# yfukasawa/LongQC

Measured on AMD Instinct MI355X. Metric: Mbases/sec all-vs-all overlap coverage (sampleqc hot path), higher is better.
Workload: dtype u64; 1 GPU; BASELINE configs[2]: 500000 synthetic PacBio Sequel CLR reads ~10 kb 30x, pb-sequel preset (-Y -l 0 -q 160 -k 12 -w 5 -I 4G -p 80), 5000 subsample queries; target_bases=5181693140, query_bases=51577117, parallelism=single GPU

## Files before the change

longqc_amd/csrc/engine.cpp:

```cpp
#include "engine.hpp"
#include "kernels_sketch.hpp"
#include "kernels_index.hpp"
#include "kernels_seed.hpp"
#include "kernels_sort.hpp"
#include "kernels_walk.hpp"
#include "kernels_psort.hpp"
#include "kernels_chain.hpp"
#include "fastx.hpp"
#include "fastx_mem.hpp"
#include "sat_replay.hpp"
#ifndef LQ_EMU
extern "C" void lq_segv_altstack();
#endif
#include <cstdio>
#include <cstring>
#include <cmath>
#include <cinttypes>
#include <algorithm>
#include <unordered_map>
#include <deque>
#include <future>
#include <functional>

static inline u32 nblk(u64 n, u32 bs)
// ... 50 lines not shown
}
void lqcov_handle::drain_stages()
{
	std::lock_guard<std::mutex> g(stage_mu);
	for (lqcov_handle::StagePending &sp : stage_pending) { hipEventSynchronize(sp.b); account_stage(sp.name, sp.a, sp.b, sp.bytes); }
	stage_pending.clear();
	for (auto &kv : late_bytes) { auto it = stages.find(kv.first); if (it != stages.end()) it->second.bytes += kv.second; }
	late_bytes.clear();
}
void lqcov_handle::add_stage_bytes(const char *name, u64 bytes)
{
	if (!profiling || !bytes) return;
	std::lock_guard<std::mutex> g(stage_mu);
	late_bytes[name] += bytes;
}

void Knobs::read_env()
{
	auto num = [](const char *name, long dflt) { const char *e = getenv(name); return e && *e ? atol(e) : dflt; };
	auto is = [](const char *name, const char *val) { const char *e = getenv(name); return e && !strcmp(e, val); };
	lanes = (int)std::min<long>(8, std::max<long>(1, num("LQCOV_LANES", 3)));
	anchor_budget = getenv("LQCOV_ANCHOR_BUDGET") ? strtoull(getenv("LQCOV_ANCHOR_BUDGET"), 0, 10) : 0;
	query_order_file = is("LQCOV_QUERY_ORDER", "file");
	query_order_striped = is("LQCOV_QUERY_ORDER", "striped");
	all_klib = is("LQCOV_SORT", "klib");
	ps_shift = (u32)std::min<long>(12, std::max<long>(0, num("LQCOV_PS_SHIFT", 0)));
	reg_walker = !is("LQCOV_WALK", "solo");
	ckpt = !is("LQCOV_CKPT", "0");
	ckpt3 = num("LQCOV_CKPT3", 1) > 0;
	sort_tile = (u32)std::max<long>(0, num("LQCOV_SORT_TILE", 0)); if (sort_tile && sort_tile < 64) sort_tile = 64;
	walk_shift = (u32)std::min<long>(16, std::max<long>(0, num("LQCOV_WALK_SHIFT", 0)));
	chain_wave_min = (int)std::max<long>(0, num("LQCOV_CHAIN_WAVE_MIN", 0));
	chain_cap = (int)num("LQCOV_CHAIN_CAP", 128);
	run_stage = (u32)std::max<long>(1, num("LQCOV_RUN_STAGE", LQ_RUN_STAGE));
	run_grid = (u32)std::max<long>(1, num("LQCOV_RUN_GRID", 2048));
	ps_key64 = num("LQCOV_PS_KEY64", 0) != 0;
	sketch_wgen = num("LQCOV_SKETCH_WGEN", 0) != 0;
	upload_amb = num("LQCOV_UPLOAD_AMB", 0) != 0;
	sketch_fast = num("LQCOV_SKETCH_FAST", 1) != 0;
#ifndef LQ_EMU
	lq_trace_launches = (int)num("LQCOV_TRACE_LAUNCHES", 0);
#endif
	no_level_skip = getenv("LQCOV_NO_LEVEL_SKIP") != nullptr;
	debug_sort = getenv("LQCOV_DEBUG_SORT") != nullptr;
	sketch_kpt = (u32)std::min<long>(64, std::max<long>(1, num("LQCOV_SKETCH_KPT", 4)));
	sketch_machine_only = is("LQCOV_SKETCH", "machine");
	upload_slices = (u32)std::min<long>(8, std::max<long>(1, num("LQCOV_UPLOAD_SLICES", 4)));
	upload_min_chunks = (u64)std::max<long>(1, num("LQCOV_UPLOAD_MIN_CHUNKS", 1L << 16));
	tile_grid = (u32)std::max<long>(64, num("LQCOV_TILE_GRID", 4096));
	ps_passes = (u32)std::min<long>(16, std::max<long>(0, num("LQCOV_PS_PASSES", 2))) & ~1u;
	ties_klib = is("LQCOV_TIES", "klib") || all_klib;
	filter = num("LQCOV_FILTER", 1) != 0;
	parse_threads = (int)std::min<long>(256, std::max<long>(0, num("LQCOV_PARSE_THREADS", 0)));
	parse_piece = (u64)std::max<long>(64, num("LQCOV_PARSE_PIECE", 32L << 20));
	parse_side = getenv("LQCOV_PARSE_SIDE") ? strtoull(getenv("LQCOV_PARSE_SIDE"), 0, 10) : 2ULL << 30;
	pipeline = num("LQCOV_PIPELINE", 1) != 0;
	plan_ahead = num("LQCOV_PLAN_AHEAD", 1) != 0;
	cnt_bits = (int)std::min<long>(16, std::max<long>(2, num("LQCOV_TEST_CNT_BITS", 16)));
	seed_bucket = (u32)std::min<long>(1L << 24, std::max<long>(16, num("LQCOV_SEED_BUCKET", 7600)));
	seed_chunk = getenv("LQCOV_SEED_CHUNK") ? std::max<u64>(1024, strtoull(getenv("LQCOV_SEED_CHUNK"), 0, 10)) : 1ULL << 30;
	if (seed_chunk > 0xfffffff0ULL) seed_chunk = 0xfffffff0ULL;
	seed_segl = (u32)std::min<long>(LQ_SD_SEGL, std::max<long>(1, num("LQCOV_SEED_SEGL", LQ_SD_SEGL)));
	seed_pair_bits = (u32)std::min<long>(LQ_SD_PAIR_BITS, std::max<long>(1, num("LQCOV_SEED_PAIR_BITS", LQ_SD_PAIR_BITS)));
	seed_hwords = (u32)std::min<long>(LQ_SD_HWORDS, std::max<long>(2, num("LQCOV_SEED_HWORDS", LQ_SD_HWORDS)));
	seed_surv_max = getenv("LQCOV_SEED_SURV_MAX") ? std::max<u64>(1, strtoull(getenv("LQCOV_SEED_SURV_MAX"), 0, 10)) : 2ULL << 30;
	seed_dcap = (u32)std::min<long>(LQ_SD_DCAP, std::max<long>(1, num("LQCOV_SEED_DCAP", LQ_SD_DCAP)));
// ... 709 lines not shown
		sort_recs.push_back(std::move(rec));
	}
	if (K.debug_sort) {
		std::vector<mm128> ha(nA);
		d2h(ha.data(), dA, nA, L.stream);
		u64 sum_after = 0;
		for (u64 i = 0; i < nA; ++i) sum_after += dbg_anchor_sum(ha[i]);
		if (sum_after != sum_before) fprintf(stderr, "[sort] batch of %u queries: NOT A PERMUTATION of the emitted anchors (sums %016llx / %016llx)\n", nqb, (unsigned long long)sum_before, (unsigned long long)sum_after);
		u64 unsorted = 0, ties = 0, unmarked = 0;
		for (u32 q = 0; q < nqb; ++q)
			for (u64 i = h_off[q] + 1; i < h_off[q + 1]; ++i) {
				if (ha[i].x < ha[i - 1].x) ++unsorted;
				if (ha[i].x == ha[i - 1].x) { ++ties; if (!(ha[i].y & LQ_TIE_MARK) || !(ha[i - 1].y & LQ_TIE_MARK)) { if (unmarked++ < 4) fprintf(stderr, "[sort] query %u of the batch: equal x %016llx, y %016llx / %016llx\n", q, (unsigned long long)ha[i].x, (unsigned long long)ha[i - 1].y, (unsigned long long)ha[i].y); } }
			}
		fprintf(stderr, "[sort] batch of %u queries: %llu anchors, %llu out of order, %llu equal-x neighbours, %llu of them with an unmarked anchor\n", nqb, (unsigned long long)nA, (unsigned long long)unsorted, (unsigned long long)ties, (unsigned long long)unmarked);
		if (sum_after != sum_before || unsorted || unmarked) throw std::logic_error("LQCOV_DEBUG_SORT: the sorted anchors are not a permutation of the emitted ones, not ascending, or hold an unmarked tie (see stderr)");
	}
}

void lqcov_handle::batch_buffers(MapLane &L, u64 nA)
{
	if (nA > 0xfffffff0ULL) throw std::domain_error("a single query produces more than 2^32 anchors against this part");
	const u64 nA4 = ((nA + 1) * 4 + 15) & ~(u64)15;
	L.A.ensure((nA + 1) * 16); L.B.ensure(std::max<u64>((nA + 1) * 16, nA4 * 4));
	L.scr.ensure(nA4 * 5 + 64);
}

void lqcov_handle::chain_stage(MapLane &L, Part &pt, const u64 *aqb, u64 a_base, u32 nqb, u32 q0, const u32 *qmap, u64 nA, int tie_mode, u32 n_want, u32 ivl_cap, bool dbg, const SatSink *sink)
{
	mm128 *dA = L.A.as<mm128>();
	const u64 nA4 = ((nA + 1) * 4 + 15) & ~(u64)15;
	u64 *d_cu = (u64*)((u8*)L.scr.p + 3 * nA4);
	i32 *d_cf = (i32*)L.B.p, *d_cp = (i32*)((u8*)L.B.p + nA4), *d_ct = (i32*)((u8*)L.B.p + 2 * nA4), *d_cv = (i32*)((u8*)L.B.p + 3 * nA4);
	u64 n_groups = 0;
	if (tie_mode == 2 && a_base == 0 && qmap) {
		L.gstart.ensure(((u64)n_want + 1) * 8);
		if (n_want) {
			StageTimer t(this, L.stream, "k_run_list", (u64)n_want * 16);
			LQ_LAUNCH(k_want_runs, nblk(n_want, 256), 256, L.stream, dA, aqb, nqb, qmap, L.want.as<unsigned long long>(), n_want, L.gstart.as<u64>()); check_launch();
		}
		n_groups = n_want;
	} else {
		const u32 n_tiles = (u32)((nA + LQ_RUN_TILE - 1) / LQ_RUN_TILE);
		const u32 n_min = run_n_min();
		L.run_tiles.ensure(16);
		L.gstart.ensure((nA / n_min + 1) * 8);
		dzero(L.run_tiles.p, 4, L.stream);
		{
			StageTimer t(this, L.stream, "k_run_list", nA * 16);
			LQ_LAUNCH(k_run_list, std::min<u32>(n_tiles, K.run_grid), LQ_RUN_THREADS, L.stream, dA, nA, aqb, a_base, nqb, n_tiles, n_min, std::max<u32>(LQ_RUN_THREADS, std::min<u32>(K.run_stage, LQ_RUN_STAGE)), L.run_tiles.as<u32>(), L.gstart.as<u64>()); check_launch();
		}
		u32 ng = 0;
		d2h(&ng, L.run_tiles.as<u32>(), 1, L.stream);
		n_groups = ng;
	}
	ChainBufs cb; cb.f = d_cf; cb.p = d_cp; cb.t = d_ct; cb.v = d_cv; cb.u = d_cu;
	CovState cs;
	cs.lambda = lambda.as<unsigned long long>(); cs.lambda2 = lambda2.as<unsigned long long>();
	cs.cnts = cnts.as<u32>(); cs.qflags = qflags.as<u32>(); cs.skip = skip.as<u32>(); cs.qmoff = cnt_off_dev();
	cs.mini_pos = mini_pos.as<u64>(); cs.mpq_off = mpq_off.as<u64>(); cs.qlen = q.d_len.as<u32>(); cs.tlen = pt.rs.d_len.as<u32>();
	cs.ivl = L.ivl.as<Ivl>(); cs.n_ivl = L.n_ivl.as<u32>(); cs.ivl_cap = ivl_cap;
	cs.dbg = dbg ? dbg_chains.as<ChainRec>() : nullptr; cs.n_dbg = n_dbg.as<unsigned long long>(); cs.dbg_cap = dbg_cap;
	cs.tie_mode = tie_mode; cs.qmap = qmap; cs.thr = have_thr ? q_thr.as<u32>() : nullptr;
	cs.cnt_max = cnt_max;
	cs.rec = sink ? sink->rec : nullptr; cs.n_rec = sink ? sink->n_rec : nullptr; cs.rec_cap = sink ? sink->rec_cap : 0;
	cs.rec_at = sink ? sink->at : nullptr; cs.n_at = sink ? sink->n_at : nullptr; cs.at_cap = sink ? sink->at_cap : 0;
	cs.sens = nullptr; cs.n_sens = L.n_sens.as<u32>(); cs.sens_cap = 0; cs.want = L.want.as<unsigned long long>(); cs.n_want = n_want;
	if (tie_mode == 1) {
		L.sens.ensure((n_groups + 1) * 8);
		cs.sens = L.sens.as<unsigned long long>(); cs.sens_cap = (u32)std::min<u64>(n_groups, 0xfffffff0ULL);
	}
	if (n_groups > 0xfffffff0ULL) throw std::domain_error("too many anchor runs in one batch");
	const int cap = K.chain_cap <= 64 ? 64 : K.chain_cap <= 128 ? 128 : 256;
	const int wave_min = tie_mode == 2 && K.chain_wave_min <= 0 ? std::min<int>(LQ_CHAIN_WAVE_MIN, std::max<int>(P.min_cnt, 8)) : std::min(cap + 1, K.chain_wave_min > 0 ? K.chain_wave_min : LQ_CHAIN_WAVE_MIN);
	if (n_groups) {
		StageTimer t(this, L.stream, "k_chain", nA * 16);
#define LQ_CHAIN_LAUNCH(CAP) LQ_LAUNCH((k_chain<CAP>), nblk(n_groups, 64), 64, L.stream, dA, L.gstart.as<u64>(), (const u32*)nullptr, (u32)n_groups, aqb, a_base, nqb, q0, avg_qspan.as<float>(), mp, cs, (i32)P.min_cnt, (i32)(wave_min - 1))
		if (cap == 64) { LQ_CHAIN_LAUNCH(64); } else if (cap == 128) { LQ_CHAIN_LAUNCH(128); } else { LQ_CHAIN_LAUNCH(256); }
#undef LQ_CHAIN_LAUNCH
		check_launch();
	}
	{
		u32 n_sel = 0;
		const u32 n_tiles = (u32)((n_groups + LQ_RUN_TILE - 1) / LQ_RUN_TILE);
		L.sel_tiles.ensure(((u64)n_tiles + 2) * 4);
		LQ_LAUNCH(k_sel_count, std::min<u32>(std::max<u32>(n_tiles, 1), 1u << 16), LQ_RUN_THREADS, L.stream, L.gstart.as<u64>(), n_groups, (i32)wave_min, (i32)0x7fffffff, n_tiles, L.sel_tiles.as<u32>()); check_launch();
		LQ_LAUNCH(k_tile_scan, 1, LQ_TSCAN_THREADS, L.stream, L.sel_tiles.as<u32>(), n_tiles); check_launch();
		d2h(&n_sel, L.sel_tiles.as<u32>() + n_tiles, 1, L.stream);
		if (n_sel) {
			L.gsel.ensure((u64)n_sel * 4); L.gkey.ensure((u64)n_sel * 4); L.gsel2.ensure((u64)n_sel * 4); L.gkey2.ensure((u64)n_sel * 4);
			LQ_LAUNCH(k_sel_write, std::min<u32>(n_tiles, 1u << 16), LQ_RUN_THREADS, L.stream, L.gstart.as<u64>(), n_groups, (i32)wave_min, (i32)0x7fffffff, n_tiles, L.sel_tiles.as<u32>(), L.gsel.as<u32>(), L.gkey.as<u32>()); check_launch();
			L.prim.sort_pairs_u32_u32(L.gkey.as<u32>(), L.gkey2.as<u32>(), L.gsel.as<u32>(), L.gsel2.as<u32>(), n_sel);
			StageTimer t(this, L.stream, "k_chain_wave");
			LQ_LAUNCH(k_chain_wave, n_sel, 64, L.stream, dA, L.gstart.as<u64>(), L.gsel2.as<u32>(), n_sel, aqb, a_base, nqb, q0, avg_qspan.as<float>(), mp, cb, cs);
			check_launch();
		}
	}
}

void lqcov_handle::sat_replay_part(Part &pt, const std::vector<u64> &h_aq, const std::vector<u64> &h_qmoff)
{
	const u32 n_q = q.n;
	if (!n_q || distributed) return;
	std::vector<u32> hf(n_q), hs(n_q);
	d2h(hf.data(), qflags.as<u32>(), n_q, stream);
	bool any = false;
	for (u32 i = 0; i < n_q; ++i) any |= (hf[i] & 1u) != 0;
	if (!any) return;
	d2h(hs.data(), skip.as<u32>(), n_q, stream);
	for (u32 qi = 0; qi < n_q; ++qi) {
		if (!(hf[qi] & 1u) || hs[qi]) continue;
		std::vector<SatRec> recs; std::vector<u32> at;
		if (!sat_chains(pt, qi, h_aq, h_qmoff, recs, at)) continue;
		MapLane &L = *lanes[0];
		u64 off[2];
		d2h(off, cnt_off_dev() + qi, 2, L.stream);
		const size_t nc = (size_t)(off[1] - off[0]);
		sat_check(recs, at, nc);
		auto it = sat_cnt.find(qi);
		if (it == sat_cnt.end()) {
			std::vector<u32> c(nc);
			d2h(c.data(), cnts.as<u32>() + off[0], nc, L.stream);
			bool ok = true;
			for (const SatRec &r : recs) if (r.good) {
				ok &= c[(size_t)r.sti] > 0; --c[(size_t)r.sti];
				for (u32 k = 0; k < r.n_at; ++k) { u32 &o = c[at[r.at_off + k]]; ok &= o > 0; --o; }
			}
			for (u32 v : c) ok &= v < cnt_max;
			if (!ok) throw std::runtime_error("replay of saturated counters: the recorded chains of query " + q.names[qi] + " do not add up to its counters");
// ... 1707 lines not shown
```

longqc_amd/csrc/engine.hpp:

```cpp
#pragma once
#include "lq_common.hpp"
#include "prim.hpp"
struct KeyMap;
struct PsData;
#include "../../include/lqcov.h"
#include <string>
#include <vector>
#include <map>
#include <memory>
#include <mutex>
#include <condition_variable>
#include <thread>
#include <atomic>
#include <exception>

struct StageAcc { double ms = 0; u64 launches = 0; u64 bytes = 0; };

struct Knobs {
	int lanes = 3;
	u64 anchor_budget = 0;
	bool query_order_striped = false;
	bool query_order_file = false;
	bool all_klib = false;
	u32 ps_shift = 0;
	bool reg_walker = true;
	bool ckpt = true, ckpt3 = true;
	u32 sort_tile = 0;
	u32 walk_shift = 0;
	int chain_wave_min = 0, chain_cap = 128;
	bool sketch_fast = true;
	bool upload_amb = false;
	bool sketch_wgen = false;
	bool ps_key64 = false;
	u32 run_grid = 2048;
	u32 run_stage = 2048;
	bool no_level_skip = false;
	bool debug_sort = false;
	u32 sketch_kpt = 4;
	u32 ps_passes = 2;
	u32 tile_grid = 4096;
	u64 upload_min_chunks = 1u << 16;
	u32 upload_slices = 4;
	bool sketch_machine_only = false;
	bool ties_klib = false;
	bool filter = true;
	bool plan_ahead = true;
	int parse_threads = 0;
	u64 parse_piece = 32u << 20;
	u64 parse_side = 2ULL << 30;
	bool pipeline = true;
	int cnt_bits = 16;
	u32 seed_bucket = 7600;
	u64 seed_chunk = 1ULL << 30;
	u32 seed_segl = 256;
	u32 seed_pair_bits = 13;
	u32 seed_dcap = 8192, seed_bigcap = 65536;
	u64 seed_surv_max = 2ULL << 30;
	u32 seed_hwords = 12288;
	void read_env();
};

struct SatSink {
	SatRec *rec; unsigned long long *n_rec; u64 rec_cap;
	u32 *at; unsigned long long *n_at; u64 at_cap;
};

// ... 332 lines not shown
```

longqc_amd/csrc/kernels_chain.hpp:

```cpp
#pragma once
#include "lq_common.hpp"
#include "kernels_sketch.hpp"
#include "kernels_sort.hpp"

#define LQ_RUN_TILE 4096
#define LQ_RUN_THREADS 256
#define LQ_RUN_ROWS (LQ_RUN_TILE / LQ_RUN_THREADS)
#define LQ_RUN_WAVES (LQ_RUN_THREADS / 64)

#define LQ_TSCAN_THREADS 1024
__global__ void __launch_bounds__(LQ_TSCAN_THREADS)
k_tile_scan(u32 *cnt, u32 n)
{
	__shared__ u32 wsum[LQ_TSCAN_THREADS / 64];
	const u32 t = threadIdx.x, lane = t & 63, w = t >> 6;
	const u32 per = (n + LQ_TSCAN_THREADS - 1) / LQ_TSCAN_THREADS;
	const u32 a = (u64)t * per < n ? t * per : n, b = a + per < n ? a + per : n;
	u32 sum = 0;
	for (u32 x = a; x < b; ++x) sum += cnt[x];
	u32 inc = sum;
	for (int d = 1; d < 64; d <<= 1) { const u32 o = __shfl_up(inc, d); if ((int)lane >= d) inc += o; }
	if (lane == 63) wsum[w] = inc;
	__syncthreads();
	if (t == 0) { u32 run = 0; for (u32 x = 0; x < LQ_TSCAN_THREADS / 64; ++x) { const u32 v = wsum[x]; wsum[x] = run; run += v; } cnt[n] = run; }
	__syncthreads();
	u32 run = wsum[w] + inc - sum;
	for (u32 x = a; x < b; ++x) { const u32 v = cnt[x]; cnt[x] = run; run += v; }
}

__device__ __forceinline__ u32 lq_hi32(const mm128 *a) { return ((const u32*)a)[1]; }
#define LQ_RUN_START(e) ((u64)(u32)(e))
#define LQ_RUN_LEN(e) ((i64)((e) >> 32))
#define LQ_RUN_STAGE 2048
#define LQ_RUN_PEEK 64
__global__ void __launch_bounds__(LQ_RUN_THREADS)
k_run_list(const mm128 *A, u64 n, const u64 *aq_off, u64 a_base, u32 n_q, u32 n_tiles, u32 n_min, u32 stage ,
           u32 *n_runs, u64 *runs)
{
	__shared__ u32 qbits[LQ_RUN_TILE / 32];
	__shared__ u32 hb[LQ_RUN_TILE / 32 + 2];
	__shared__ u32 nx[LQ_RUN_PEEK];
	__shared__ u32 slot0, fill_s;
	__shared__ u64 stg[LQ_RUN_STAGE];
	const u32 t = threadIdx.x, lane = t & 63;
	const u32 per = (n_tiles + gridDim.x - 1) / gridDim.x;
	const u32 T0 = blockIdx.x * per < n_tiles ? blockIdx.x * per : n_tiles, T1 = T0 + per < n_tiles ? T0 + per : n_tiles;
	const u64 near_mask = n_min > 1 ? (n_min > 33 ? ~0ULL >> 31 : (1ULL << (n_min - 1)) - 1) : 0;
	u32 qlo = ~0u;
	if (t < 2) hb[LQ_RUN_TILE / 32 + t] = 0;
	if (t == 0) fill_s = 0;
	__syncthreads();
#define LQ_RUN_FLUSH(f) do { \
		if (t == 0) { slot0 = atomicAdd(n_runs, (f)); } \
		__syncthreads(); \
		for (u32 i_ = t; i_ < (f); i_ += LQ_RUN_THREADS) runs[slot0 + i_] = stg[i_]; \
		if (t == 0) { fill_s = 0; } \
		__syncthreads(); } while (0)
	for (u32 T = T0; T < T1; ++T) {
		const u64 base = (u64)T * LQ_RUN_TILE;
		const u32 tl = n - base < LQ_RUN_TILE ? (u32)(n - base) : LQ_RUN_TILE;
		if (t < LQ_RUN_PEEK) nx[t] = base + tl + t < n ? lq_hi32(A + base + tl + t) : 0u;
		if (t < LQ_RUN_TILE / 32) qbits[t] = 0;
		__syncthreads();
		{
			u32 lo = qlo, hi = n_q;
			if (lo == ~0u) { lo = 0; while (hi - lo > 1) { const u32 mid = lo + ((hi - lo) >> 1); if (aq_off[mid] - a_base <= base) lo = mid; else hi = mid; } }
			else while (lo + 1 < n_q && aq_off[lo + 1] - a_base <= base) ++lo;
			qlo = lo;
			for (u32 q = lo + t; q < n_q; q += LQ_RUN_THREADS) {
				const u64 p = aq_off[q] - a_base;
				if (p >= base + LQ_RUN_TILE) break;
				if (p >= base && aq_off[q] < aq_off[q + 1]) atomicOr(&qbits[(u32)(p - base) >> 5], 1u << ((u32)(p - base) & 31));
			}
		}
		__syncthreads();
		const u32 *hp = (const u32*)(A + base) + 1;
#pragma unroll 1
		for (u32 j0 = 0; j0 < LQ_RUN_ROWS; j0 += 8) {
			u32 h[8];
#pragma unroll
			for (u32 j = 0; j < 8; ++j) { const u32 o = (j0 + j) * LQ_RUN_THREADS + t; h[j] = o < tl ? hp[4 * o] : 0u; }
#pragma unroll
			for (u32 j = 0; j < 8; ++j) {
// ... 21 lines not shown
			}
			const u32 o = j * LQ_RUN_THREADS + t;
			u32 len = 0;
			if (hb[o >> 5] >> (o & 31) & 1) {
				const u32 w0 = (o + 1) >> 5, sh = (o + 1) & 31;
				const u64 win = (((u64)hb[w0 + 1] << 32 | hb[w0]) >> sh) | (sh ? (u64)hb[w0 + 2] << (64 - sh) : 0);
				if ((win & near_mask) == 0) {
					u32 nxt = LQ_RUN_TILE;
					if (win) nxt = o + 1 + (u32)__builtin_ctzll(win);
					else {
						for (u32 wi = w0 + 2; wi < LQ_RUN_TILE / 32; ++wi) { const u32 m = hb[wi]; if (m) { nxt = wi * 32 + (u32)__builtin_ctz(m); break; } }
					}
					if (nxt < tl) len = nxt - o;
					else if (base + tl >= n) len = tl - o;
					else {
						u32 q = qlo;
						while (aq_off[q + 1] - a_base <= base + o) ++q;
						const u64 qend = aq_off[q + 1] - a_base;
						const u32 h = lq_hi32(A + base + o);
						u64 lo = base + tl, hi = qend;
						const u32 pk = hi - lo < LQ_RUN_PEEK ? (u32)(hi - lo) : LQ_RUN_PEEK;
						u32 i = 0;
						while (i < pk && nx[i] == h) ++i;
						lo += i;
						if (i == LQ_RUN_PEEK)
							while (lo < hi) { const u64 mid = lo + ((hi - lo) >> 1); if (lq_hi32(A + mid) == h) lo = mid + 1; else hi = mid; }
						len = (u32)(lo - (base + o));
					}
				}
			}
			const bool viable = len >= n_min && len != 0;
			const u64 vb = __ballot(viable);
			if (vb) {
				u32 b = 0;
				if (lane == 0) b = atomicAdd(&fill_s, (u32)__popcll(vb));
				b = __shfl(b, 0);
				if (viable) stg[b + (u32)__popcll(vb & ((1ULL << lane) - 1))] = (base + o) | (u64)len << 32;
			}
		}
		__syncthreads();
	}
	{
		const u32 f = fill_s;
		__syncthreads();
		if (f) LQ_RUN_FLUSH(f);
	}
#undef LQ_RUN_FLUSH
}

__device__ __forceinline__ int lq_ilog2_32(u32 v) { return 31 - __clz(v); }

template <class UP>
__device__ __forceinline__ void lq_heapsort_u64(UP a, i64 n)
{
	if (n < 2) return;
	for (i64 start = n / 2 - 1; start >= 0; --start) {
		i64 root = start; u64 v = a[root];
		for (;;) {
			i64 ch = 2 * root + 1;
			if (ch >= n) break;
			if (ch + 1 < n && a[ch + 1] > a[ch]) ++ch;
			if (a[ch] <= v) break;
			a[root] = a[ch]; root = ch;
		}
		a[root] = v;
	}
	for (i64 end = n - 1; end > 0; --end) {
		u64 v = a[end]; a[end] = a[0];
		i64 root = 0;
		for (;;) {
			i64 ch = 2 * root + 1;
			if (ch >= end) break;
			if (ch + 1 < end && a[ch + 1] > a[ch]) ++ch;
			if (a[ch] <= v) break;
			a[root] = a[ch]; root = ch;
		}
		a[root] = v;
	}
// ... 33 lines not shown
	if (a.x >> 63) x = qlen - 1 - (x + 1 - q_span);
	return x;
}

struct ChainBufs {
	i32 *f, *p, *t, *v;
	u64 *u;
};

struct CovState {
	unsigned long long *lambda, *lambda2;
	u32 *cnts;
	u32 *qflags;
	const u32 *skip;
	const u64 *qmoff;
	const u64 *mini_pos;
	const u64 *mpq_off;
	const u32 *qlen;
	const u32 *tlen;
	Ivl *ivl; u32 *n_ivl; u32 ivl_cap;
	ChainRec *dbg; unsigned long long *n_dbg; u64 dbg_cap;
	int tie_mode;
	unsigned long long *sens; u32 *n_sens; u32 sens_cap;
	const unsigned long long *want; u32 n_want;
	const u32 *qmap;
	const u32 *thr;
	u32 cnt_max;
	SatRec *rec; unsigned long long *n_rec; u64 rec_cap; u32 *rec_at; unsigned long long *n_at; u64 at_cap;
};

__device__ __forceinline__ i32 lq_sc_med(const MapParams &P, const CovState &C, u32 q) { return C.thr ? (i32)(C.thr[q] >> 16) : (i32)(u16)P.min_sc_med; }
__device__ __forceinline__ i32 lq_sc_good(const MapParams &P, const CovState &C, u32 q) { return C.thr ? (i32)(C.thr[q] & 0xffffu) : (i32)(u16)P.min_sc_good; }

__device__ __forceinline__ bool lq_tie_wanted(const CovState &C, u32 q, u32 hi)
{
	const unsigned long long key = (unsigned long long)q << 32 | hi;
	u32 lo = 0, n = C.n_want;
	while (lo < n) { const u32 mid = lo + ((n - lo) >> 1); if (C.want[mid] < key) lo = mid + 1; else n = mid; }
	return lo < C.n_want && C.want[lo] == key;
}
#define LQ_TIE_WHY_BREAK 4u
#define LQ_TIE_WHY_PEAK 5u
__device__ __forceinline__ void lq_tie_list(const CovState &C, u32 q, u32 hi, u32 why)
{
	atomicAdd(C.n_sens + (why >= 1u && why <= 5u ? why : 6u), 1u);
	const u32 s = atomicAdd(C.n_sens, 1u);
	if (s < C.sens_cap) C.sens[s] = (unsigned long long)q << 32 | hi;
}

__global__ void __launch_bounds__(LQ_RUN_THREADS)
k_sel_count(const u64 *gstart, u64 n_groups, i32 min_cnt, i32 max_cnt, u32 n_tiles, u32 *tile_cnt)
{
	__shared__ u32 tot;
	for (u32 T = blockIdx.x; T < n_tiles; T += gridDim.x) {
		if (threadIdx.x == 0) tot = 0;
		__syncthreads();
		u32 c = 0;
		for (int j = 0; j < LQ_RUN_ROWS; ++j) {
			const u64 g = (u64)T * LQ_RUN_TILE + (u32)j * LQ_RUN_THREADS + threadIdx.x;
			i64 l = 0;
			if (g < n_groups) l = LQ_RUN_LEN(gstart[g]);
			c += (u32)__popcll(__ballot(g < n_groups && l >= (i64)min_cnt && l <= (i64)max_cnt));
		}
		if ((threadIdx.x & 63) == 0) atomicAdd(&tot, c);
		__syncthreads();
		if (threadIdx.x == 0) tile_cnt[T] = tot;
		__syncthreads();
// ... 234 lines not shown
	}
	return false;
}

__global__ void k_want_runs(const mm128 *A, const u64 *aq_off, u32 n_q, const u32 *qmap, const unsigned long long *want, u32 n_want, u64 *gstart)
{
	const u32 w = blockIdx.x * blockDim.x + threadIdx.x;
	if (w >= n_want) return;
	const u32 q = (u32)(want[w] >> 32), hi = (u32)want[w];
	u32 lo = 0, n = n_q;
	while (lo < n) { const u32 mid = lo + ((n - lo) >> 1); if (qmap[mid] < q) lo = mid + 1; else n = mid; }
	u64 e = 0;
	if (lo < n_q && qmap[lo] == q) {
		const u64 s1 = aq_off[lo + 1];
		u64 a = aq_off[lo], b = s1;
		while (a < b) { const u64 m = a + ((b - a) >> 1); if (lq_hi32(A + m) < hi) a = m + 1; else b = m; }
		u64 c = a, d = s1;
		while (c < d) { const u64 m = c + ((d - c) >> 1); if (lq_hi32(A + m) <= hi) c = m + 1; else d = m; }
		e = a | (c - a) << 32;
	}
	gstart[w] = e;
}

template <class AP, class IP, class UP>
__device__ __forceinline__ void lq_chain_run(AP a, const i64 n, IP f, IP p, IP t, IP v, UP u,
                                             const u32 q, const bool accumulate, const float *avg_qspan_q, const MapParams &P, const CovState &C)
{
	const bool watch = C.tie_mode == 1;
	u32 why = lq_chain_fill(a, n, f, p, t, v, avg_qspan_q[q], P, watch);
	if (!why && lq_chain_finish(a, n, f, p, t, v, u, q, accumulate, P, C, watch)) why = LQ_TIE_WHY_PEAK;
	if (why) lq_tie_list(C, q, (u32)(a[0].x >> 32), why);
}

template <class AP>
__device__ __forceinline__ bool lq_run_viable(AP a, i64 n, const MapParams &P)
{
	if (n < P.min_cnt) return false;
	if (n * 255 < P.min_sc) return false;
	i64 tot = 0;
	for (i64 i = 0; i < n && tot < P.min_sc; ++i) tot += (i64)(a[i].y >> 32 & 0xff);
	return tot >= P.min_sc;
}

template <int LQ_CHAIN_LDS_CAP>
__global__ void __launch_bounds__(64)
k_chain(const mm128 *A, const u64 *gstart, const u32 *glist, u32 n_list, const u64 *aq_off, u64 a_base, u32 n_q, u32 q0,
        const float *avg_qspan_q, MapParams P, CovState C, i32 min_len, i32 max_len)
{
	LQ_SHARED mm128 s_a[LQ_CHAIN_LDS_CAP];
	LQ_SHARED i32 s_f[LQ_CHAIN_LDS_CAP], s_p[LQ_CHAIN_LDS_CAP], s_t[LQ_CHAIN_LDS_CAP], s_v[LQ_CHAIN_LDS_CAP];
	LQ_SHARED u64 s_u[LQ_CHAIN_LDS_CAP];
	LQ_SHARED u32 s_n[64], s_q[64], s_done[64];
	const u32 gi0 = blockIdx.x * blockDim.x;
	LQ_BLOCK_LOOP(ln) {
		u32 todo = 0;
		const u32 gi = gi0 + ln;
		if (gi < n_list) {
			const u32 g = glist ? glist[gi] : gi;
			const u64 gs = LQ_RUN_START(gstart[g]);
			const i64 n = LQ_RUN_LEN(gstart[g]);
			if (n >= min_len && n <= max_len && n <= LQ_CHAIN_LDS_CAP && lq_run_viable(A + gs, n, P)) {
				const u32 qi = lq_find_seg(aq_off, n_q, gs + a_base);
				const u32 q = C.qmap ? C.qmap[qi] : q0 + qi;
				if ((!C.skip[q] || C.dbg) && (C.tie_mode != 2 || lq_tie_wanted(C, q, lq_hi32(A + gs)))) { todo = (u32)n; s_q[ln] = q; }
			}
		}
		s_n[ln] = todo; s_done[ln] = 0;
	}
// ... 187 lines not shown
				const u32 o2 = atomicAdd(&cn[at], 1u);
				if (o2 + 1 >= C.cnt_max) atomicOr(&C.qflags[q], 1u);
			}
		}
	}
	return false;
}

__device__ __forceinline__ void lq_wave_replay(const WaveCand *cand, i32 *st_sh, i64 cnt, bool more_beyond, bool watch, i32 max_skip)
{
	i32 max_f = st_sh[0], max_j = st_sh[1], n_skip = st_sh[2], done = 0;
	TieGroup tg; tg.x = (u32)st_sh[5]; tg.m = st_sh[6]; tg.top = st_sh[7]; tg.st = (u32)st_sh[8];
	for (i64 c = 0; c < cnt; ++c) {
		const WaveCand w = cand[c];
		if (!(w.flags & 1)) continue;
		if (watch) { const u32 why = tg.see(w.x32, w.sc, (w.flags & 2) != 0, max_f, n_skip); if (why && !st_sh[4]) st_sh[4] = (i32)why; }
		if (w.sc > max_f) { max_f = w.sc; max_j = w.j; if (n_skip > 0) --n_skip; }
		else if (w.flags & 2) {
			if (++n_skip > max_skip) {
				if (watch) {
					i64 c2 = c + 1;
					for (; c2 < cnt && cand[c2].x32 == w.x32; ++c2) if ((cand[c2].flags & 1) && tg.raises(cand[c2].sc) && !st_sh[4]) st_sh[4] = (i32)LQ_TIE_WHY_BREAK;
					if (c2 == cnt && more_beyond && !st_sh[4]) st_sh[4] = (i32)LQ_TIE_WHY_BREAK;
				}
				done = 1; break;
			}
		}
	}
	if (watch && (done || !more_beyond) && tg.bad() && !st_sh[4]) st_sh[4] = (i32)tg.why();
	st_sh[0] = max_f; st_sh[1] = max_j; st_sh[2] = n_skip; st_sh[3] = done;
	st_sh[5] = (i32)tg.x; st_sh[6] = tg.m; st_sh[7] = tg.top; st_sh[8] = (i32)tg.st;
}

__global__ void __launch_bounds__(64)
k_chain_wave(const mm128 *A, const u64 *gstart, const u32 *glist, u32 n_list, const u64 *aq_off, u64 a_base, u32 n_q, u32 q0,
             const float *avg_qspan_q, MapParams P, ChainBufs B, CovState C)
{
	LQ_SHARED WaveCand cand[64];
	LQ_SHARED i32 st_sh[10];
	LQ_SHARED i32 stamp[64];
	if (blockIdx.x >= n_list) return;
	const u32 g = glist[blockIdx.x];
	const u64 gs = LQ_RUN_START(gstart[g]);
	const i64 n = LQ_RUN_LEN(gstart[g]);
	const mm128 *a = A + gs;
	if (!lq_run_viable(a, n, P)) return;
	const u32 qi_ = lq_find_seg(aq_off, n_q, gs + a_base);
	const u32 q = C.qmap ? C.qmap[qi_] : q0 + qi_;
	const bool accumulate = !C.skip[q];
	if (!accumulate && !C.dbg) return;
	if (C.tie_mode == 2 && !lq_tie_wanted(C, q, lq_hi32(a))) return;
	const bool watch = C.tie_mode == 1;
	const u32 ln = threadIdx.x;
	if (ln == 0) st_sh[4] = 0;
	stamp[ln] = -1;
	i32 *f = B.f + gs, *p = B.p + gs, *t = B.t + gs, *v = B.v + gs;
	u64 *u = B.u + gs;
	const float avg_qspan = avg_qspan_q[q];
	const i32 max_dist = P.max_gap, bw = P.bw, max_skip = P.max_skip;
	for (i64 i = ln; i < n; i += 64) t[i] = 0;
	LQ_BLOCK_SYNC();
	const u32 n32 = (u32)n, x_hi = lq_hi32(a);
	u32 st = 0;
	u32 wx = 0; i32 wy = 0, wf = 0, wp = -1, wv = 0;
	mm128 cur = a[ln < n32 ? ln : n32 - 1], nxt = a[64 + ln < n32 ? 64 + ln : n32 - 1];
	for (u32 i = 0; i < n32; ++i) {
		const u32 bi = i & 63;
		if (bi == 0 && i) { cur = nxt; const u32 k2 = i + 64 + ln; nxt = a[k2 < n32 ? k2 : n32 - 1]; }
		const u32 rx = (u32)LQ_WAVE_LANE((u32)cur.x, bi);
		const i32 qi = LQ_WAVE_LANE((u32)cur.y, bi), q_span = LQ_WAVE_LANE((u32)(cur.y >> 32), bi) & 0xff;
		const u64 ri = (u64)x_hi << 32 | rx;
		const i32 j = (i32)i - 1 - (i32)ln;
		{
			const u64 far = __ballot(j >= 0 && rx - wx > (u32)max_dist);
			if (far) { const u32 s2 = i - (u32)__builtin_ctzll(far); if (s2 > st) st = s2; }
			else while (st + 64 < i && ri - a[st].x > (u64)max_dist) ++st;
		}
		i32 max_f = q_span, max_j = -1, n_skip = 0, done = 0;
		bool active = false; i32 sc = 0;
		if (j >= (i32)st) {
			const i64 dr = (i64)(rx - wx);
			const i32 dq = qi - wy;
			if (!(dr == 0 || dq <= 0 || dq > max_dist)) {
				const i32 dd = dr > dq ? (i32)(dr - dq) : (i32)(dq - dr);
				if (dd <= bw) {
					const i32 min_d = dq < dr ? dq : (i32)dr;
					sc = min_d > q_span ? q_span : min_d;
					const i32 log_dd = dd ? lq_ilog2_32((u32)dd) : 0;
					sc -= (i32)((double)dd * .01 * (double)avg_qspan) + (log_dd >> 1);
					sc += wf;
					active = true;
					if (wp >= 0) { if (wp + 64 >= (i32)i) stamp[wp & 63] = (i32)i; else t[wp] = (i32)i; }
// ... 42 lines not shown
			if (ln == 0) { st_sh[0] = max_f; st_sh[1] = max_j; st_sh[2] = 0; st_sh[3] = 0; st_sh[8] = 0; }
			LQ_WAVE_SYNC();
			if (ln == 0) lq_wave_replay(cand, st_sh, i - st < 64 ? i - st : 64, more, watch, max_skip);
			LQ_WAVE_SYNC();
			max_f = st_sh[0]; max_j = st_sh[1]; n_skip = st_sh[2]; done = st_sh[3];
		}
		bool beyond = false;
		if (!done && more) {
			LQ_BLOCK_SYNC();
			if (ln == 0) { st_sh[0] = max_f; st_sh[1] = max_j; st_sh[2] = n_skip; st_sh[3] = 0; if (!serial) st_sh[8] = 0; }
			LQ_BLOCK_SYNC();
			for (i64 top = (i64)i - 65; top >= (i64)st; top -= 64) {
				const i64 jj = top - (i64)ln;
				i32 c_sc = 0, c_flags = 0; u32 c_x32 = 0;
				if (jj >= (i64)st) {
					const mm128 aj = a[jj];
					c_x32 = (u32)aj.x;
					const i64 dr = (i64)(ri - aj.x);
					const i32 dq = qi - (i32)aj.y;
					if (!(dr == 0 || dq <= 0 || dq > max_dist)) {
						const i32 dd = dr > dq ? (i32)(dr - dq) : (i32)(dq - dr);
						if (dd <= bw) {
							const i32 min_d = dq < dr ? dq : (i32)dr;
							i32 s2 = min_d > q_span ? q_span : min_d;
							const i32 log_dd = dd ? lq_ilog2_32((u32)dd) : 0;
							s2 -= (i32)((double)dd * .01 * (double)avg_qspan) + (log_dd >> 1);
							c_sc = s2 + f[jj];
							c_flags = 1;
							const i32 pj = p[jj];
							if (pj >= 0) t[pj] = (i32)i;
						}
					}
				}
				cand[ln].sc = c_sc; cand[ln].j = (i32)jj; cand[ln].flags = c_flags; cand[ln].x32 = c_x32;
				LQ_BLOCK_SYNC();
				if (cand[ln].flags & 1) { if (t[cand[ln].j] == (i32)i) cand[ln].flags |= 2; }
				LQ_BLOCK_SYNC();
				if (ln == 0) lq_wave_replay(cand, st_sh, top - (i64)st + 1 < 64 ? top - (i64)st + 1 : 64, top - 64 >= (i64)st, watch, max_skip);
				LQ_BLOCK_SYNC();
				if (st_sh[3]) break;
			}
			max_f = st_sh[0]; max_j = st_sh[1];
			LQ_BLOCK_SYNC();
			beyond = true;
		}
		if (watch && (serial || beyond) && st_sh[4]) break;
		i32 vi = max_f;
		if (max_j >= 0) {
			const u32 back = i - 1 - (u32)max_j;
			if (back >= 64) LQ_BLOCK_SYNC();
			const i32 vj = back < 64 ? LQ_WAVE_LANE(wv, back) : v[max_j];
			if (vj > max_f) vi = vj;
		}
		wx = (u32)lq_wave_shr1((i32)wx, (i32)rx); wy = lq_wave_shr1(wy, qi); wf = lq_wave_shr1(wf, max_f); wp = lq_wave_shr1(wp, max_j); wv = lq_wave_shr1(wv, vi);
		if (bi == 63 || i + 1 == n32) {
			if (ln <= bi) { const u32 k = i - ln; f[k] = wf; p[k] = wp; v[k] = wv; }
		}
	}
	LQ_BLOCK_SYNC();
	const bool listed = st_sh[4] != 0;
	LQ_BLOCK_SYNC();
	if (C.rec) {
		if (ln == 0) lq_chain_finish(a, n, f, p, t, v, u, q, accumulate, P, C, false);
		return;
	}
	const bool peak_tie = !listed && lq_chain_finish_wave(a, n, f, p, t, v, u, q, accumulate, P, C, watch, st_sh);
	if (ln == 0 && (listed || peak_tie)) lq_tie_list(C, q, lq_hi32(a), listed ? (u32)st_sh[4] : LQ_TIE_WHY_PEAK);
}

__global__ void k_ivl_offsets(const u32 *qkey, u32 n_ivl, u32 n_q, u32 *ivq_off)
{
	u32 q = blockIdx.x * blockDim.x + threadIdx.x;
	if (q > n_q) return;
	u32 lo = 0, hi = n_ivl;
	while (lo < hi) { u32 mid = lo + ((hi - lo) >> 1); if (qkey[mid] < q) lo = mid + 1; else hi = mid; }
	ivq_off[q] = lo;
}

__global__ void k_filter_redundant(const u64 *se , const u32 *ivq_off, u32 n_q, u32 min_cov,
                                   u32 *scratch , Ivl *pv, u32 *n_pv, u32 pv_cap)
{
	u32 q = blockIdx.x * blockDim.x + threadIdx.x;
	if (q >= n_q) return;
	const u32 lo = ivq_off[q], n = ivq_off[q + 1] - lo;
	if (n == 0) return;
	const u64 *cv = se + lo;
	u32 *vc = scratch + (u64)lo * 4, *mc = vc + 2 * (u64)n;
	for (u32 i = 0; i < n; ++i) { vc[2 * i] = (u32)cv[i]; vc[2 * i + 1] = (u32)(cv[i] >> 32); }
	lq_heapsort_u32(vc, 2 * (i64)n);
	u32 med_start = 0, med_cov = 0, n_mc = 0;
	for (u32 j = 0; j < 2 * n; ++j) {
		const u32 e = vc[j], old = med_cov;
		if (e & 2) {
			if (e & 1) { if (e & 4) med_cov -= min_cov; else --med_cov; }
			else       { if (e & 4) med_cov += min_cov; else ++med_cov; }
		}
		if (old < min_cov && med_cov >= min_cov) med_start = e;
		else if (old >= min_cov && med_cov < min_cov) {
			const u32 mlen = (e >> 3) - med_start;
			if (mlen > 0) {
// ... 111 lines not shown
```

Measured before the change: 15320 Mbases/s.

## Remove host syncs in wave chaining and replace serial replay with wave scans

k_run_list now also counts long runs, so the host can size the selection buffers from that count. This removes a device-to-host read of the selected count before the wave-chain launch, and the kernels read the count from device memory instead. k_chain_wave is split into a compute kernel with a grid-stride loop and lighter arguments, plus a separate finish kernel, which is meant to cut register pressure. In non-watch mode the single-lane serial candidate replay is replaced by wave-wide max and compose scans, removing several block syncs for each 64-candidate step. The trade-offs are an extra launch, extra run-state buffers, and more complex scan logic that has to reproduce the replay semantics exactly.

```diff
diff --git a/longqc_amd/csrc/engine.cpp b/longqc_amd/csrc/engine.cpp
--- a/longqc_amd/csrc/engine.cpp
+++ b/longqc_amd/csrc/engine.cpp
@@ -106,6 +106,7 @@
 	walk_shift = (u32)std::min<long>(16, std::max<long>(0, num("LQCOV_WALK_SHIFT", 0)));
 	chain_wave_min = (int)std::max<long>(0, num("LQCOV_CHAIN_WAVE_MIN", 0));
 	chain_cap = (int)num("LQCOV_CHAIN_CAP", 128);
+	chain_wave_grid = (u32)std::min<long>(1L << 20, std::max<long>(1, num("LQCOV_CHAIN_WAVE_GRID", 1L << 20)));
 	run_stage = (u32)std::max<long>(1, num("LQCOV_RUN_STAGE", LQ_RUN_STAGE));
 	run_grid = (u32)std::max<long>(1, num("LQCOV_RUN_GRID", 2048));
 	ps_key64 = num("LQCOV_PS_KEY64", 0) != 0;
@@ -881,7 +882,11 @@
 	const u64 nA4 = ((nA + 1) * 4 + 15) & ~(u64)15;
 	u64 *d_cu = (u64*)((u8*)L.scr.p + 3 * nA4);
 	i32 *d_cf = (i32*)L.B.p, *d_cp = (i32*)((u8*)L.B.p + nA4), *d_ct = (i32*)((u8*)L.B.p + 2 * nA4), *d_cv = (i32*)((u8*)L.B.p + 3 * nA4);
+	const int cap = K.chain_cap <= 64 ? 64 : K.chain_cap <= 128 ? 128 : 256;
+	const int wave_min = tie_mode == 2 && K.chain_wave_min <= 0 ? std::min<int>(LQ_CHAIN_WAVE_MIN, std::max<int>(P.min_cnt, 8)) : std::min(cap + 1, K.chain_wave_min > 0 ? K.chain_wave_min : LQ_CHAIN_WAVE_MIN);
 	u64 n_groups = 0;
+	u32 n_long = 0;
+	bool n_long_exact = false;
 	if (tie_mode == 2 && a_base == 0 && qmap) {
 		L.gstart.ensure(((u64)n_want + 1) * 8);
 		if (n_want) {
@@ -889,19 +894,21 @@
 			LQ_LAUNCH(k_want_runs, nblk(n_want, 256), 256, L.stream, dA, aqb, nqb, qmap, L.want.as<unsigned long long>(), n_want, L.gstart.as<u64>()); check_launch();
 		}
 		n_groups = n_want;
+		n_long = n_want;
 	} else {
 		const u32 n_tiles = (u32)((nA + LQ_RUN_TILE - 1) / LQ_RUN_TILE);
 		const u32 n_min = run_n_min();
 		L.run_tiles.ensure(16);
 		L.gstart.ensure((nA / n_min + 1) * 8);
-		dzero(L.run_tiles.p, 4, L.stream);
+		dzero(L.run_tiles.p, 8, L.stream);
 		{
 			StageTimer t(this, L.stream, "k_run_list", nA * 16);
-			LQ_LAUNCH(k_run_list, std::min<u32>(n_tiles, K.run_grid), LQ_RUN_THREADS, L.stream, dA, nA, aqb, a_base, nqb, n_tiles, n_min, std::max<u32>(LQ_RUN_THREADS, std::min<u32>(K.run_stage, LQ_RUN_STAGE)), L.run_tiles.as<u32>(), L.gstart.as<u64>()); check_launch();
-		}
-		u32 ng = 0;
-		d2h(&ng, L.run_tiles.as<u32>(), 1, L.stream);
-		n_groups = ng;
+			LQ_LAUNCH(k_run_list, std::min<u32>(n_tiles, K.run_grid), LQ_RUN_THREADS, L.stream, dA, nA, aqb, a_base, nqb, n_tiles, n_min, std::max<u32>(LQ_RUN_THREADS, std::min<u32>(K.run_stage, LQ_RUN_STAGE)), (u32)wave_min, L.run_tiles.as<u32>(), L.gstart.as<u64>()); check_launch();
+		}
+		u32 ng[2] = { 0, 0 };
+		d2h(ng, L.run_tiles.as<u32>(), 2, L.stream);
+		n_groups = ng[0];
+		n_long = ng[1]; n_long_exact = true;
 	}
 	ChainBufs cb; cb.f = d_cf; cb.p = d_cp; cb.t = d_ct; cb.v = d_cv; cb.u = d_cu;
 	CovState cs;
@@ -920,8 +927,6 @@
 		cs.sens = L.sens.as<unsigned long long>(); cs.sens_cap = (u32)std::min<u64>(n_groups, 0xfffffff0ULL);
 	}
 	if (n_groups > 0xfffffff0ULL) throw std::domain_error("too many anchor runs in one batch");
-	const int cap = K.chain_cap <= 64 ? 64 : K.chain_cap <= 128 ? 128 : 256;
-	const int wave_min = tie_mode == 2 && K.chain_wave_min <= 0 ? std::min<int>(LQ_CHAIN_WAVE_MIN, std::max<int>(P.min_cnt, 8)) : std::min(cap + 1, K.chain_wave_min > 0 ? K.chain_wave_min : LQ_CHAIN_WAVE_MIN);
 	if (n_groups) {
 		StageTimer t(this, L.stream, "k_chain", nA * 16);
 #define LQ_CHAIN_LAUNCH(CAP) LQ_LAUNCH((k_chain<CAP>), nblk(n_groups, 64), 64, L.stream, dA, L.gstart.as<u64>(), (const u32*)nullptr, (u32)n_groups, aqb, a_base, nqb, q0, avg_qspan.as<float>(), mp, cs, (i32)P.min_cnt, (i32)(wave_min - 1))
@@ -929,21 +934,25 @@
 #undef LQ_CHAIN_LAUNCH
 		check_launch();
 	}
-	{
-		u32 n_sel = 0;
+	if (n_long) {
 		const u32 n_tiles = (u32)((n_groups + LQ_RUN_TILE - 1) / LQ_RUN_TILE);
 		L.sel_tiles.ensure(((u64)n_tiles + 2) * 4);
 		LQ_LAUNCH(k_sel_count, std::min<u32>(std::max<u32>(n_tiles, 1), 1u << 16), LQ_RUN_THREADS, L.stream, L.gstart.as<u64>(), n_groups, (i32)wave_min, (i32)0x7fffffff, n_tiles, L.sel_tiles.as<u32>()); check_launch();
 		LQ_LAUNCH(k_tile_scan, 1, LQ_TSCAN_THREADS, L.stream, L.sel_tiles.as<u32>(), n_tiles); check_launch();
-		d2h(&n_sel, L.sel_tiles.as<u32>() + n_tiles, 1, L.stream);
-		if (n_sel) {
-			L.gsel.ensure((u64)n_sel * 4); L.gkey.ensure((u64)n_sel * 4); L.gsel2.ensure((u64)n_sel * 4); L.gkey2.ensure((u64)n_sel * 4);
-			LQ_LAUNCH(k_sel_write, std::min<u32>(n_tiles, 1u << 16), LQ_RUN_THREADS, L.stream, L.gstart.as<u64>(), n_groups, (i32)wave_min, (i32)0x7fffffff, n_tiles, L.sel_tiles.as<u32>(), L.gsel.as<u32>(), L.gkey.as<u32>()); check_launch();
-			L.prim.sort_pairs_u32_u32(L.gkey.as<u32>(), L.gkey2.as<u32>(), L.gsel.as<u32>(), L.gsel2.as<u32>(), n_sel);
-			StageTimer t(this, L.stream, "k_chain_wave");
-			LQ_LAUNCH(k_chain_wave, n_sel, 64, L.stream, dA, L.gstart.as<u64>(), L.gsel2.as<u32>(), n_sel, aqb, a_base, nqb, q0, avg_qspan.as<float>(), mp, cb, cs);
-			check_launch();
-		}
+		L.gsel.ensure((u64)n_long * 4); L.gkey.ensure((u64)n_long * 4); L.gsel2.ensure((u64)n_long * 4); L.gkey2.ensure((u64)n_long * 4);
+		if (!n_long_exact) { LQ_HIP_CHECK(hipMemsetAsync(L.gkey.p, 0xff, (size_t)n_long * 4, L.stream)); dzero(L.gsel.p, (size_t)n_long * 4, L.stream); }
+		LQ_LAUNCH(k_sel_write, std::min<u32>(n_tiles, 1u << 16), LQ_RUN_THREADS, L.stream, L.gstart.as<u64>(), n_groups, (i32)wave_min, (i32)0x7fffffff, n_tiles, L.sel_tiles.as<u32>(), L.gsel.as<u32>(), L.gkey.as<u32>()); check_launch();
+		L.prim.sort_pairs_u32_u32(L.gkey.as<u32>(), L.gkey2.as<u32>(), L.gsel.as<u32>(), L.gsel2.as<u32>(), n_long);
+		ChainWaveArgs wa;
+		wa.min_cnt = mp.min_cnt; wa.min_sc = mp.min_sc; wa.max_gap = mp.max_gap; wa.bw = mp.bw; wa.max_skip = mp.max_skip;
+		wa.tie_mode = cs.tie_mode; wa.n_want = cs.n_want; wa.dbg = cs.dbg ? 1u : 0u; wa.qmap = cs.qmap; wa.skip = cs.skip; wa.want = cs.want;
+		const u32 grid = std::min<u32>(n_long, K.chain_wave_grid);
+		const u32 *n_sel = L.sel_tiles.as<u32>() + n_tiles;
+		StageTimer t(this, L.stream, "k_chain_wave");
+		LQ_LAUNCH(k_chain_wave, grid, 64, L.stream, dA, L.gstart.as<u64>(), L.gsel2.as<u32>(), n_sel, aqb, a_base, nqb, q0, avg_qspan.as<float>(), cb, wa, L.gsel.as<u32>(), L.gkey.as<u32>());
+		check_launch();
+		LQ_LAUNCH(k_chain_wave_finish, grid, 64, L.stream, dA, L.gstart.as<u64>(), L.gsel2.as<u32>(), n_sel, mp, cb, cs, L.gsel.as<u32>(), L.gkey.as<u32>());
+		check_launch();
 	}
 }
 
diff --git a/longqc_amd/csrc/engine.hpp b/longqc_amd/csrc/engine.hpp
--- a/longqc_amd/csrc/engine.hpp
+++ b/longqc_amd/csrc/engine.hpp
@@ -32,6 +32,7 @@
 	bool upload_amb = false;
 	bool sketch_wgen = false;
 	bool ps_key64 = false;
+	u32 chain_wave_grid = 1u << 20;
 	u32 run_grid = 2048;
 	u32 run_stage = 2048;
 	bool no_level_skip = false;
diff --git a/longqc_amd/csrc/kernels_chain.hpp b/longqc_amd/csrc/kernels_chain.hpp
--- a/longqc_amd/csrc/kernels_chain.hpp
+++ b/longqc_amd/csrc/kernels_chain.hpp
@@ -35,12 +35,12 @@
 #define LQ_RUN_PEEK 64
 __global__ void __launch_bounds__(LQ_RUN_THREADS)
 k_run_list(const mm128 *A, u64 n, const u64 *aq_off, u64 a_base, u32 n_q, u32 n_tiles, u32 n_min, u32 stage ,
-           u32 *n_runs, u64 *runs)
+           u32 n_long , u32 *n_runs, u64 *runs)
 {
 	__shared__ u32 qbits[LQ_RUN_TILE / 32];
 	__shared__ u32 hb[LQ_RUN_TILE / 32 + 2];
 	__shared__ u32 nx[LQ_RUN_PEEK];
-	__shared__ u32 slot0, fill_s;
+	__shared__ u32 slot0, fill_s, long_s;
 	__shared__ u64 stg[LQ_RUN_STAGE];
 	const u32 t = threadIdx.x, lane = t & 63;
 	const u32 per = (n_tiles + gridDim.x - 1) / gridDim.x;
@@ -48,7 +48,7 @@
 	const u64 near_mask = n_min > 1 ? (n_min > 33 ? ~0ULL >> 31 : (1ULL << (n_min - 1)) - 1) : 0;
 	u32 qlo = ~0u;
 	if (t < 2) hb[LQ_RUN_TILE / 32 + t] = 0;
-	if (t == 0) fill_s = 0;
+	if (t == 0) { fill_s = 0; long_s = 0; }
 	__syncthreads();
 #define LQ_RUN_FLUSH(f) do { \
 		if (t == 0) { slot0 = atomicAdd(n_runs, (f)); } \
@@ -136,6 +136,8 @@
 			const bool viable = len >= n_min && len != 0;
 			const u64 vb = __ballot(viable);
 			if (vb) {
+				const u64 lb = __ballot(viable && len >= n_long);
+				if (lane == 0 && lb) atomicAdd(&long_s, (u32)__popcll(lb));
 				u32 b = 0;
 				if (lane == 0) b = atomicAdd(&fill_s, (u32)__popcll(vb));
 				b = __shfl(b, 0);
@@ -148,6 +150,7 @@
 		const u32 f = fill_s;
 		__syncthreads();
 		if (f) LQ_RUN_FLUSH(f);
+		if (t == 0 && long_s) atomicAdd(n_runs + 1, long_s);
 	}
 #undef LQ_RUN_FLUSH
 }
@@ -247,7 +250,8 @@
 __device__ __forceinline__ i32 lq_sc_med(const MapParams &P, const CovState &C, u32 q) { return C.thr ? (i32)(C.thr[q] >> 16) : (i32)(u16)P.min_sc_med; }
 __device__ __forceinline__ i32 lq_sc_good(const MapParams &P, const CovState &C, u32 q) { return C.thr ? (i32)(C.thr[q] & 0xffffu) : (i32)(u16)P.min_sc_good; }
 
-__device__ __forceinline__ bool lq_tie_wanted(const CovState &C, u32 q, u32 hi)
+template <class CP >
+__device__ __forceinline__ bool lq_tie_wanted(const CP &C, u32 q, u32 hi)
 {
 	const unsigned long long key = (unsigned long long)q << 32 | hi;
 	u32 lo = 0, n = C.n_want;
@@ -548,8 +552,8 @@
 	if (why) lq_tie_list(C, q, (u32)(a[0].x >> 32), why);
 }
 
-template <class AP>
-__device__ __forceinline__ bool lq_run_viable(AP a, i64 n, const MapParams &P)
+template <class AP, class PP>
+__device__ __forceinline__ bool lq_run_viable(AP a, i64 n, const PP &P)
 {
 	if (n < P.min_cnt) return false;
 	if (n * 255 < P.min_sc) return false;
@@ -803,32 +807,36 @@
 	st_sh[5] = (i32)tg.x; st_sh[6] = tg.m; st_sh[7] = tg.top; st_sh[8] = (i32)tg.st;
 }
 
-__global__ void __launch_bounds__(64)
-k_chain_wave(const mm128 *A, const u64 *gstart, const u32 *glist, u32 n_list, const u64 *aq_off, u64 a_base, u32 n_q, u32 q0,
-             const float *avg_qspan_q, MapParams P, ChainBufs B, CovState C)
-{
-	LQ_SHARED WaveCand cand[64];
-	LQ_SHARED i32 st_sh[10];
-	LQ_SHARED i32 stamp[64];
-	if (blockIdx.x >= n_list) return;
-	const u32 g = glist[blockIdx.x];
-	const u64 gs = LQ_RUN_START(gstart[g]);
-	const i64 n = LQ_RUN_LEN(gstart[g]);
+struct ChainWaveArgs {
+	i32 min_cnt, min_sc, max_gap, bw, max_skip;
+	int tie_mode;
+	u32 n_want, dbg;
+	const u32 *qmap, *skip;
+	const unsigned long long *want;
+};
+#define LQ_WAVE_RUN_NONE 0xffffffffu
+
+__device__ __forceinline__ u32 lq_chain_wave_run(const mm128 *A, const u64 e, const u64 *aq_off, u64 a_base, u32 n_q, u32 q0, const float *avg_qspan_q,
+                                                 const ChainBufs &B, const ChainWaveArgs &W, WaveCand *cand, i32 *st_sh, i32 *stamp, u32 &q_out)
+{
+	const u64 gs = LQ_RUN_START(e);
+	const i64 n = LQ_RUN_LEN(e);
 	const mm128 *a = A + gs;
-	if (!lq_run_viable(a, n, P)) return;
+	if (!lq_run_viable(a, n, W)) return LQ_WAVE_RUN_NONE;
 	const u32 qi_ = lq_find_seg(aq_off, n_q, gs + a_base);
-	const u32 q = C.qmap ? C.qmap[qi_] : q0 + qi_;
-	const bool accumulate = !C.skip[q];
-	if (!accumulate && !C.dbg) return;
-	if (C.tie_mode == 2 && !lq_tie_wanted(C, q, lq_hi32(a))) return;
-	const bool watch = C.tie_mode == 1;
+	const u32 q = W.qmap ? W.qmap[qi_] : q0 + qi_;
+	const bool accumulate = !W.skip[q];
+	if (!accumulate && !W.dbg) return LQ_WAVE_RUN_NONE;
+	const int tie_mode = W.tie_mode;
+	if (tie_mode == 2 && !lq_tie_wanted(W, q, lq_hi32(a))) return LQ_WAVE_RUN_NONE;
+	q_out = q;
+	const bool watch = tie_mode == 1;
 	const u32 ln = threadIdx.x;
 	if (ln == 0) st_sh[4] = 0;
 	stamp[ln] = -1;
 	i32 *f = B.f + gs, *p = B.p + gs, *t = B.t + gs, *v = B.v + gs;
-	u64 *u = B.u + gs;
 	const float avg_qspan = avg_qspan_q[q];
-	const i32 max_dist = P.max_gap, bw = P.bw, max_skip = P.max_skip;
+	const i32 max_dist = W.max_gap, bw = W.bw, max_skip = W.max_skip;
 	for (i64 i = ln; i < n; i += 64) t[i] = 0;
 	LQ_BLOCK_SYNC();
 	const u32 n32 = (u32)n, x_hi = lq_hi32(a);
@@ -937,6 +945,26 @@
 						}
 					}
 				}
+				if (!watch) {
+					LQ_BLOCK_SYNC();
+					const bool c_act = c_flags != 0;
+					const bool c_tm = c_act && t[jj] == (i32)i;
+					const i32 inc = lq_wave_scan_max(c_act ? c_sc : (i32)0x80000000);
+					i32 exc = lq_wave_shr1(inc, (i32)0x80000000);
+					if (exc < max_f) exc = max_f;
+					const bool rec = c_act && c_sc > exc;
+					const bool skp = c_act && !rec && c_tm;
+					i32 fa = rec ? -1 : skp ? 1 : 0, fb = rec ? 0 : -(1 << 29);
+					lq_wave_scan_compose(fa, fb);
+					const i32 x_after = n_skip + fa > fb ? n_skip + fa : fb;
+					const u64 brk = __ballot(skp && x_after > max_skip);
+					const u32 cb = brk ? (u32)__builtin_ctzll(brk) : 64u;
+					const u64 recm = __ballot(rec) & (cb >= 63 ? ~0ULL : (2ULL << cb) - 1);
+					if (recm) { const int last = 63 - __clzll(recm); max_f = LQ_WAVE_LANE(c_sc, last); max_j = (i32)top - last; }
+					n_skip = LQ_WAVE_LANE(x_after, 63);
+					if (cb < 64) break;
+					continue;
+				}
 				cand[ln].sc = c_sc; cand[ln].j = (i32)jj; cand[ln].flags = c_flags; cand[ln].x32 = c_x32;
 				LQ_BLOCK_SYNC();
 				if (cand[ln].flags & 1) { if (t[cand[ln].j] == (i32)i) cand[ln].flags |= 2; }
@@ -945,7 +973,7 @@
 				LQ_BLOCK_SYNC();
 				if (st_sh[3]) break;
 			}
-			max_f = st_sh[0]; max_j = st_sh[1];
+			if (watch) { max_f = st_sh[0]; max_j = st_sh[1]; }
 			LQ_BLOCK_SYNC();
 			beyond = true;
 		}
@@ -963,14 +991,51 @@
 		}
 	}
 	LQ_BLOCK_SYNC();
-	const bool listed = st_sh[4] != 0;
+	const u32 why = (u32)st_sh[4];
 	LQ_BLOCK_SYNC();
-	if (C.rec) {
-		if (ln == 0) lq_chain_finish(a, n, f, p, t, v, u, q, accumulate, P, C, false);
-		return;
-	}
-	const bool peak_tie = !listed && lq_chain_finish_wave(a, n, f, p, t, v, u, q, accumulate, P, C, watch, st_sh);
-	if (ln == 0 && (listed || peak_tie)) lq_tie_list(C, q, lq_hi32(a), listed ? (u32)st_sh[4] : LQ_TIE_WHY_PEAK);
+	return why | (accumulate ? 256u : 0u);
+}
+
+__global__ void __launch_bounds__(64)
+k_chain_wave(const mm128 *A, const u64 *gstart, const u32 *glist, const u32 *n_list, const u64 *aq_off, u64 a_base, u32 n_q, u32 q0,
+             const float *avg_qspan_q, ChainBufs B, ChainWaveArgs W, u32 *run_q, u32 *run_st)
+{
+	LQ_SHARED WaveCand cand[64];
+	LQ_SHARED i32 st_sh[10];
+	LQ_SHARED i32 stamp[64];
+	const u32 n_l = *n_list;
+	for (u32 b = blockIdx.x; b < n_l; b += gridDim.x) {
+		u32 q = 0;
+		const u32 r = lq_chain_wave_run(A, gstart[glist[b]], aq_off, a_base, n_q, q0, avg_qspan_q, B, W, cand, st_sh, stamp, q);
+		if (threadIdx.x == 0) { run_q[b] = q; run_st[b] = r; }
+		LQ_BLOCK_SYNC();
+	}
+}
+
+__global__ void __launch_bounds__(64)
+k_chain_wave_finish(const mm128 *A, const u64 *gstart, const u32 *glist, const u32 *n_list, MapParams P, ChainBufs B, CovState C, const u32 *run_q, const u32 *run_st)
+{
+	LQ_SHARED i32 sh[8];
+	const u32 n_l = *n_list;
+	for (u32 b = blockIdx.x; b < n_l; b += gridDim.x) {
+		const u32 r = run_st[b];
+		if (r == LQ_WAVE_RUN_NONE) continue;
+		const u32 q = run_q[b], why = r & 255u;
+		const bool accumulate = (r & 256u) != 0;
+		const u64 e = gstart[glist[b]];
+		const u64 gs = LQ_RUN_START(e);
+		const i64 n = LQ_RUN_LEN(e);
+		const mm128 *a = A + gs;
+		i32 *f = B.f + gs, *p = B.p + gs, *t = B.t + gs, *v = B.v + gs;
+		u64 *u = B.u + gs;
+		if (C.rec) {
+			if (threadIdx.x == 0) lq_chain_finish(a, n, f, p, t, v, u, q, accumulate, P, C, false);
+		} else {
+			const bool peak_tie = !why && lq_chain_finish_wave(a, n, f, p, t, v, u, q, accumulate, P, C, C.tie_mode == 1, sh);
+			if (threadIdx.x == 0 && (why || peak_tie)) lq_tie_list(C, q, lq_hi32(a), why ? why : LQ_TIE_WHY_PEAK);
+		}
+		LQ_BLOCK_SYNC();
+	}
 }
 
 __global__ void k_ivl_offsets(const u32 *qkey, u32 n_ivl, u32 n_q, u32 *ivq_off)
```

Result: faster. 15790 Mbases/s, median of 6 (+3.1%).
